# OSU-slatelab/ASR-CRaFT

Hardware: AMD Instinct MI355X
Metric: utterances/sec SCRF forward-backward (TIMIT-shape) (higher is better)
Workload: dtype f64; 1 GPU; BASELINE config 2: segmental CRF forward-backward, 48 labels, max-seg-len 25, 39-dim x 300-frame utterances, stdstate map (lambda_len 18528); global_minibatch=4096, precision=fastlin, parallelism=dp1, rccl_ranks=0

## Files before the change

### asr-craft_amd/csrc/scrf_engine.cpp

```cpp
#include <dlfcn.h>
#include <time.h>
#include <unistd.h>
#include <stdarg.h>
#include <stdio.h>
#include <stdlib.h>
#include <string.h>

#include <algorithm>
#include <cmath>
#include <string>
#include <unordered_map>
#include <vector>

#include "scrf_kernels.h"

typedef struct { char internal[128]; } scrf_nccl_uid;
typedef void* scrf_nccl_comm;
struct RcclApi {
  void* lib = nullptr;
  int (*GetUniqueId)(scrf_nccl_uid*) = nullptr;
  int (*CommInitRank)(scrf_nccl_comm*, int, scrf_nccl_uid, int) = nullptr;
  int (*AllReduce)(const void*, void*, size_t, int, int, scrf_nccl_comm, hipStream_t) = nullptr;
  int (*CommDestroy)(scrf_nccl_comm) = nullptr;
  int (*GroupStart)() = nullptr;
// ... 55 lines not shown
  bool m0_valid = false;
  double* d_sums = nullptr;
  double* d_stage = nullptr;
  double* d_lamT[2] = {nullptr, nullptr};
  double* d_sums_stage = nullptr;
  int* d_latch = nullptr;
  int* h_latch = nullptr;
  double* h_sums = nullptr;
  hipEvent_t ev_sums = nullptr;
  bool sums_queued = false;
  hipEvent_t ev_status = nullptr;
  uint64_t n_lin_fallback = 0;
  char* scratch = nullptr;
  size_t scratch_cap = 0;
  hipStream_t stream2 = nullptr;
  struct PoolBlock { void* p; size_t cap; uint64_t epoch; };
  std::vector<PoolBlock> pool_free;
  std::unordered_map<void*, size_t> pool_cap;
  hipStream_t up_stream = nullptr;
  hipEvent_t pool_ev[8] = {nullptr, nullptr, nullptr, nullptr, nullptr, nullptr, nullptr, nullptr};
  uint64_t pool_epoch = 0, pool_done = 0;
  size_t pool_bytes = 0;
  char* scratch2 = nullptr;
  size_t scratch2_cap = 0;
  double* d_grad2 = nullptr;
  double* d_sums2 = nullptr;
  hipEvent_t ev_fork = nullptr, ev_join = nullptr;
  bool overlap_comm = false;
  bool early_done = false;
  uint64_t n_collectives = 0, n_overlapped = 0;
  double* d_pack = nullptr;
  void* d_rtab = nullptr;
  size_t rtab_bytes = 0;
  double* d_dtab = nullptr;
  double* d_sl_tab = nullptr;
  bool frame_mass = false;
  uint64_t n_post_split = 0, n_post_whole = 0;
  bool force_fb = false;
  double* d_w1 = nullptr;
  uint64_t n_decode_fix = 0, n_decode_fallback = 0;
  uint32_t *dec_lab = nullptr, *dec_n = nullptr, *dec_hlab = nullptr, *dec_hn = nullptr;
  float *dec_cost = nullptr, *dec_hcost = nullptr;
  uint64_t dec_cap_f = 0, dec_cap_u = 0;
  char* post_buf = nullptr;
  size_t post_cap = 0;
  scrf_arc* lp_arcs = nullptr;
  uint64_t lp_cap = 0;
  char* lp_meta = nullptr;
  size_t lp_meta_cap = 0;
  scrf_batch lp_batch = nullptr;
  std::vector<uint64_t> lp_off;
  uint64_t n_lp_calls = 0, n_lp_chunks = 0;
  uint32_t* al_ph = nullptr;
  uint64_t* al_off = nullptr;
  uint64_t al_cap_ph = 0, al_cap_u = 0;
  std::vector<uint64_t> al_bp_off;
  uint64_t n_al_calls = 0, n_al_chunks = 0, n_al_wave = 0, n_al_group = 0;
  uint32_t* tr_inv = nullptr;
  uint64_t tr_cap_inv = 0;
  std::vector<uint64_t> tr_cell_off;
  std::vector<uint32_t> tr_inv_h;
  uint64_t n_tr_calls = 0, n_tr_chunks = 0, n_tr_redone = 0;
  std::string err;
  struct KTime { std::string name; double ms; uint32_t n; };
  std::vector<KTime> ktimes;
  hipEvent_t kev[2] = {nullptr, nullptr};
// ... 187 lines not shown
  size_t nb = sizeof(double) * lay.lambda_len;
  CRCHK(hipMalloc((void**)&h->d_lambda, nb));
  CRCHK(hipMalloc((void**)&h->d_lambda_acc, nb));
  CRCHK(hipMalloc((void**)&h->d_gsa, nb));
  CRCHK(hipMalloc((void**)&h->d_grad, nb));
  CRCHK(hipMalloc((void**)&h->d_m0, sizeof(double) * lay.L * lay.L));
  CRCHK(hipMalloc((void**)&h->d_w1, sizeof(double) * lay.L));
  if (lay.D <= 40) CRCHK(hipMalloc((void**)&h->d_dtab, sizeof(double) * fused_dur_table_doubles(lay)));
  if (cfg->map_type >= SCRF_STDSPARSE) {
    if (lay.nsfe + lay.use_sb) CRCHK(hipMalloc((void**)&h->d_lamT[0], sizeof(double) * ((size_t)lay.nsfe + lay.use_sb) * lay.L));
    if (lay.ntfe + lay.use_tb) CRCHK(hipMalloc((void**)&h->d_lamT[1], sizeof(double) * ((size_t)lay.ntfe + lay.use_tb) * lay.L * lay.L));
  }
  if (cfg->model_type == SCRF_STDSEG && !lay.use_tf) CRCHK(hipMalloc((void**)&h->d_sl_tab, sizeof(double) * (2 * (size_t)lay.L * lay.L + 8)));
  CRCHK(hipMalloc((void**)&h->d_e0, sizeof(double) * lay.L * lay.L));
  CRCHK(hipMalloc((void**)&h->d_et0, sizeof(double) * lay.L * lay.L));
  CRCHK(hipMalloc((void**)&h->d_msh0, sizeof(double)));
  CRCHK(hipMalloc((void**)&h->d_sums, sizeof(double) * 8));
  CRCHK(hipMalloc((void**)&h->d_stage, nb));
  CRCHK(hipMalloc((void**)&h->d_sums_stage, sizeof(double) * 4));
  CRCHK(hipMalloc((void**)&h->d_latch, sizeof(int) * 2));
  CRCHK(hipHostMalloc((void**)&h->h_latch, sizeof(int) * 2, hipHostMallocDefault));
  h->h_latch[0] = h->h_latch[1] = 0;
  CRCHK(hipHostMalloc((void**)&h->h_sums, sizeof(double) * 4, hipHostMallocDefault));
  CRCHK(hipEventCreateWithFlags(&h->ev_sums, hipEventDisableTiming));
  CRCHK(hipEventCreateWithFlags(&h->ev_status, hipEventDisableTiming));
  CRCHK(hipEventCreate(&h->kev[0]));
  CRCHK(hipEventCreate(&h->kev[1]));
  CRCHK(hipMalloc((void**)&h->d_grad2, nb));
  CRCHK(hipMalloc((void**)&h->d_sums2, sizeof(double) * 4));
  CRCHK(hipStreamCreateWithFlags(&h->stream2, hipStreamNonBlocking));
  CRCHK(hipStreamCreateWithFlags(&h->up_stream, hipStreamNonBlocking));
  CRCHK(hipEventCreateWithFlags(&h->ev_fork, hipEventDisableTiming));
  CRCHK(hipEventCreateWithFlags(&h->ev_join, hipEventDisableTiming));
  CRCHK(hipMemsetAsync(h->d_lambda, 0, nb, h->stream));
  CRCHK(hipMemsetAsync(h->d_lambda_acc, 0, nb, h->stream));
  CRCHK(hipMemsetAsync(h->d_gsa, 0, nb, h->stream));
  CRCHK(hipMemsetAsync(h->d_grad, 0, nb, h->stream));
  CRCHK(hipMemsetAsync(h->d_sums, 0, sizeof(double) * 8, h->stream));
  for (int i = 0; i <= SCRF_N_PHASES; i++) {
    CRCHK(hipEventCreate(&h->ev[i][0]));
    CRCHK(hipEventCreate(&h->ev[i][1]));
  }
  h->ev_ok = true;
  CRCHK(hipStreamSynchronize(h->stream));
  if (h->shadow) {
    std::vector<double> z(h->xlay.lambda_len, 0.0);
    if (scrf_set_lambda(h, z.data(), h->xlay.lambda_len) != SCRF_OK) { g_create_err = h->err; scrf_destroy(h); return SCRF_ERR_HIP; }
  }
#undef CRCHK
  *out = h;
  return SCRF_OK;
}

extern "C" int scrf_destroy(scrf_handle h) {
  if (!h) return SCRF_OK;
  hipSetDevice(h->device);
  if (h->stream) hipStreamSynchronize(h->stream);
  if (h->comm && g_rccl.CommDestroy) g_rccl.CommDestroy(h->comm);
  hipFree(h->d_lambda); hipFree(h->d_lambda_acc); hipFree(h->d_gsa);
  if (h->own_grad) hipFree(h->d_grad);
  hipFree(h->d_grad2); hipFree(h->d_sums2); hipFree(h->scratch2);
  hipFree(h->d_stage); hipFree(h->d_sums_stage); hipFree(h->d_latch);
  hipFree(h->d_lamT[0]); hipFree(h->d_lamT[1]);
  if (h->h_latch) hipHostFree(h->h_latch);
  if (h->h_sums) hipHostFree(h->h_sums);
  if (h->ev_sums) hipEventDestroy(h->ev_sums);
  if (h->ev_status) hipEventDestroy(h->ev_status);
  if (h->kev[0]) hipEventDestroy(h->kev[0]);
  if (h->kev[1]) hipEventDestroy(h->kev[1]);
  if (h->stream2) { hipStreamSynchronize(h->stream2); hipStreamDestroy(h->stream2); }
  if (h->up_stream) { hipStreamSynchronize(h->up_stream); hipStreamDestroy(h->up_stream); }
  for (auto& bl : h->pool_free) hipFree(bl.p);
  for (auto& kv : h->pool_cap) hipFree(kv.first);
  for (int i = 0; i < 8; i++) if (h->pool_ev[i]) hipEventDestroy(h->pool_ev[i]);
  if (h->ev_fork) hipEventDestroy(h->ev_fork);
  if (h->ev_join) hipEventDestroy(h->ev_join);
  hipFree(h->dec_lab); hipFree(h->dec_n); hipFree(h->dec_cost);
  hipFree(h->al_ph); hipFree(h->al_off);
  hipFree(h->tr_inv);
  hipFree(h->post_buf);
  hipFree(h->lp_arcs); hipFree(h->lp_meta);
  if (h->dec_hlab) hipHostFree(h->dec_hlab);
  if (h->dec_hn) hipHostFree(h->dec_hn);
  if (h->dec_hcost) hipHostFree(h->dec_hcost);
  hipFree(h->d_w1); hipFree(h->d_dtab); hipFree(h->d_rtab); hipFree(h->d_pack); hipFree(h->d_sl_tab); hipFree(h->d_m0); hipFree(h->d_e0); hipFree(h->d_et0); hipFree(h->d_msh0); hipFree(h->d_sums); hipFree(h->scratch);
  if (h->ev_ok)
    for (int i = 0; i <= SCRF_N_PHASES; i++) { hipEventDestroy(h->ev[i][0]); hipEventDestroy(h->ev[i][1]); }
  if (h->own_stream && h->stream) hipStreamDestroy(h->stream);
  delete h;
  return SCRF_OK;
}

extern "C" const char* scrf_last_error(scrf_handle h) { return h ? h->err.c_str() : g_create_err.c_str(); }

extern "C" int scrf_set_stream(scrf_handle h, void* s) {
  if (!h) return SCRF_ERR_INVALID;
  HIPCHK(h, hipSetDevice(h->device));
  HIPCHK(h, hipStreamSynchronize(h->stream));
  if (h->own_stream) { hipStreamDestroy(h->stream); h->own_stream = false; }
  if (s) {
    h->stream = (hipStream_t)s;
  } else {
    HIPCHK(h, hipStreamCreateWithFlags(&h->stream, hipStreamNonBlocking));
    h->own_stream = true;
  }
  return SCRF_OK;
}

extern "C" int scrf_synchronize(scrf_handle h) {
// ... 834 lines not shown
    KT_RUN("k_windows", st, launch_windows(st, b->d_frames[s], b->d_sframe_off[s], bv, u0, u1, nfr, r.in_width, l.D, r.left_ctx, r.right_ctx,
                                           r.extract_seg_ftr, X, hybrid ? hybrid_row_floats(l, r.in_width) : l.F, col,
                                           (first_only ? 1 : 0) | (hybrid ? 2 : 0)));
  }
}

static bool ensure_m0(scrf_handle h, hipStream_t st) {
  if (h->m0_valid) return false;
  const ScrfLayout& l = h->lay;
  launch_scores_exact(st, nullptr, l.F, nullptr, 1, h->d_lambda, l, 1, l.L * l.L, h->d_m0);
  launch_exp_m(st, h->kn, h->d_m0, l.L, 1, h->d_e0, h->d_et0, h->d_msh0);
  h->m0_valid = true;
  return true;
}

static void relay_sparse_lambda(scrf_handle h, hipStream_t st) {
  launch_sp_relay(st, h->d_lambda, h->lay, 0, h->d_lamT[0]);
  if (h->lay.use_tf) launch_sp_relay(st, h->d_lambda, h->lay, 1, h->d_lamT[1]);
}

static int run_scores(scrf_handle h, scrf_batch b, uint32_t u0, uint32_t u1, ChunkBufs& cb, bool fast = false, int f32 = 0) {
  const ScrfLayout& l = h->lay;
  const uint64_t nfr = b->frame_off[u1] - b->frame_off[u0], nseg = b->seg_off[u1] - b->seg_off[u0];
  ScrfBatchView bv = b->view();
  if (cb.fused) {
    PhaseTimer tm(h, PH_SCORE, cb.st);
    const uint32_t W0 = b->recipe[0].in_width;
    ScrfFusedArgs fa = fused_args(h, b, u0, 0);
    if (h->d_dtab && h->kn.dtab) {
      launch_dur_table(cb.st, l, W0, h->d_lambda, h->d_dtab);
      fa.dtab = h->d_dtab;
      const size_t nb = fused_tile_table_bytes(l.D, fa.TB);
      if (nb > h->rtab_bytes) {
        hipFree(h->d_rtab); h->d_rtab = nullptr; h->rtab_bytes = 0;
        HIPCHK(h, hipMalloc(&h->d_rtab, nb));
        h->rtab_bytes = nb;
      }
      launch_tile_tables(cb.st, l.D, fa.TB, (cb.la && !cb.Wn) ? 1 : 0, h->d_rtab);
      if (h->kn.rtab) fa.rtab = h->d_rtab;
      fa.dma = h->kn.scores_dma ? 1 : 0;
    }
    if (pframe_supported(W0)) {
      KT_RUN("k_pframe", cb.st, launch_pframe(cb.st, b->d_frames[0] + b->frame_off[u0] * W0, W0, nfr, h->d_lambda, l, (cb.la ? 6 : 5) * l.L, cb.P));
      if (cb.la) KT_RUN("k_avg_prefix", cb.st, launch_avg_prefix(cb.st, bv, u0, u1 - u0, l.L, cb.P));
    } else {
      KT_RUN("k_scores_mfma(samples)", cb.st, launch_scores_mfma(cb.st, h->kn, b->d_frames[0] + b->frame_off[u0] * W0, W0, nullptr, nfr, h->d_lambda, l,
                         spec_samples(W0), (cb.la ? 6 : 5) * l.L, cb.P));
      if (cb.la) KT_RUN("k_avg_prefix", cb.st, launch_avg_prefix(cb.st, bv, u0, u1 - u0, l.L, cb.P));
    }
    if (cb.Wn) {
      launch_state_l1(cb.st, h->d_lambda, l, h->d_w1);
      HIPCHK(h, hipMemsetAsync(cb.fix_cnt, 0, sizeof(uint32_t), cb.st));
      ScrfDecodeOut dz;
      dz.wneg = cb.Wn; dz.w1 = h->d_w1; dz.xm_f = b->d_xm_f + b->frame_off[u0];
      dz.cnt = cb.fix_cnt; dz.list = cb.fix_list; dz.cap = cb.fix_cap;
      dz.bound_scale = h->kn.decode_bound_scale * 1.01 * 0x1p-53 * (double)(l.nsfe + 1 + 3 * W0 + 8);
      PhaseTimer tk(h, PH_K_SCORE, cb.st);
      KT_RUN("k_scores_fused(decode)", cb.st, launch_scores_fused_decode(cb.st, fa, l, h->d_lambda, cb.P, b->tile_off[0][u1] - b->tile_off[0][u0], dz));
      tk.stop(1);
      tm.stop(3);
      HIPCHK(h, hipGetLastError());
      return SCRF_OK;
    }
    cb.es_ready = cb.lin && l.L <= 48;
    {
      PhaseTimer tk(h, PH_K_SCORE, cb.st);
      KT_RUN("k_scores_fused", cb.st, launch_scores_fused(cb.st, fa, l, h->d_lambda, cb.P, b->tile_off[0][u1] - b->tile_off[0][u0], cb.S, f32,
                          cb.es_ready ? cb.smax : nullptr, cb.s_true, b->d_labels, cb.la ? 1 : 0));
      tk.stop(1);
    }
    tm.stop(2);
// ... 24 lines not shown
    KT_RUN("k_sp_scores(state)", cb.st, launch_sp_scores(cb.st, cb.X, l.F, nullptr, nseg, h->d_lamT[0], l, 0, cb.S));
    tk.stop(2);
    nl += 1;
    if (l.use_tf) {
      if (!cb.lamT_ready) launch_sp_relay(cb.st, h->d_lambda, l, 1, h->d_lamT[1]);
      launch_frame_rows(cb.st, bv, u0, u1, l.D, nfr, cb.xrow_cur, 0);
      KT_RUN("k_sp_scores(trans)", cb.st, launch_sp_scores(cb.st, cb.X, l.F, cb.xrow_cur, nfr, h->d_lamT[1], l, 1, cb.M));
      nl += 3;
    }
  } else if (!cb.fused) {
    PhaseTimer tk(h, PH_K_SCORE, cb.st);
    if (fast) KT_RUN("k_scores_mfma(state)", cb.st, launch_scores_mfma(cb.st, h->kn, cb.X, l.F, nullptr, nseg, h->d_lambda, l, scrf_spec_state(l), l.L, cb.S, f32));
    else KT_RUN("k_scores_exact(state)", cb.st, launch_scores_exact(cb.st, cb.X, l.F, nullptr, nseg, h->d_lambda, l, 0, l.L, cb.S));
    tk.stop(1);
  }
  if (sparse(h)) {
    if (!l.use_tf && ensure_m0(h, cb.st)) nl += 2;
  } else if (segtrans(h)) {
    if (fast) KT_RUN("k_scores_mfma(trans)", cb.st, launch_scores_mfma(cb.st, h->kn, cb.X, l.F, nullptr, nseg, h->d_lambda, l, scrf_spec_trans(l), l.L * l.L, cb.M, f32));
    else KT_RUN("k_scores_exact(trans)", cb.st, launch_scores_exact(cb.st, cb.X, l.F, nullptr, nseg, h->d_lambda, l, 1, l.L * l.L, cb.M));
    launch_zero_initial_rows(cb.st, bv, b->d_frame_u, u0, nfr, l.D, l.L, cb.M);
    nl += 2;
  } else if (l.use_tf) {
    launch_frame_rows(cb.st, bv, u0, u1, l.D, nfr, cb.xrow_cur, 0);
    if (fast) KT_RUN("k_scores_mfma(trans)", cb.st, launch_scores_mfma(cb.st, h->kn, cb.X, l.F, cb.xrow_cur, nfr, h->d_lambda, l, scrf_spec_trans(l), l.L * l.L, cb.M, f32));
    else KT_RUN("k_scores_exact(trans)", cb.st, launch_scores_exact(cb.st, cb.X, l.F, cb.xrow_cur, nfr, h->d_lambda, l, 1, l.L * l.L, cb.M));
    nl += 2;
  } else if (ensure_m0(h, cb.st)) nl += 2;
  tm.stop(nl);
  HIPCHK(h, hipGetLastError());
  return SCRF_OK;
}

static int run_dp(scrf_handle h, scrf_batch b, uint32_t u0, uint32_t u1, ChunkBufs& cb, bool post, uint32_t* nl_out, bool ponly = false) {
  const ScrfLayout& l = h->lay;
  const uint64_t nutt = u1 - u0, nfr = b->frame_off[u1] - b->frame_off[u0];
  const int frame_model = h->cfg.model_type == SCRF_STDFRAME || h->frame_mass;
  ScrfBatchView bv = b->view();
  uint32_t nl = 0;
  if (segtrans(h)) {
    if (fb_segtrans_smem_bytes(l, fb_block_threads(l)) > 160 * 1024)
      return fail(h, SCRF_ERR_INVALID, "labels x maximum duration = %u x %u is too large for the stdseg_no_dur recursion "
                  "(its three [D][L] rings must fit 160 KB of LDS)", l.L, l.D);
    KT_RUN("k_fb_segtrans", cb.st, launch_fb_segtrans(cb.st, h->kn, l, bv, u0, (uint32_t)nutt, b->d_prev_lab, cb.S, cb.M, cb.AD, cb.alpha, cb.beta,
                       post ? cb.XI : nullptr, b->d_numer, b->d_zx, b->d_status, post ? 1 : 0));
    nl = 1;
  } else if (!cb.wave) {
    if (fb_smem_bytes(l, fb_block_threads(l)) > 160 * 1024)
      return fail(h, SCRF_ERR_INVALID, "labels x maximum duration = %u x %u is too large for the workgroup-per-utterance recursion "
                  "(its two [D][L] rings must fit 160 KB of LDS; the wavefront kernels cover L <= 256 with D <= 40)", l.L, l.D);
    if (post && cb.xi_acc) HIPCHK(h, hipMemsetAsync(cb.xi_acc, 0, sizeof(double) * nutt * l.L * l.L, cb.st));
    KT_RUN("k_fb", cb.st, launch_fb(cb.st, l, bv, u0, (uint32_t)nutt, cb.S, cb.M, cb.m_per_frame, cb.AD, cb.alpha, cb.beta, post ? cb.XI : nullptr,
              post ? cb.xi_acc : nullptr, b->d_numer, b->d_zx, b->d_status, post ? 1 : 0, frame_model));
    nl = 1;
  } else {
    if (cb.m_per_frame) { KT_RUN("k_exp_m", cb.st, launch_exp_m(cb.st, h->kn, cb.M, l.L, nfr, cb.E, cb.ET, cb.msh)); nl++; }
    if (cb.lin) {
      const uint64_t nseg = b->seg_off[u1] - b->seg_off[u0];
      if (!cb.es_ready) {
        if (!ponly) KT_RUN("k_true_scores", cb.st, launch_true_scores(cb.st, l, bv, b->d_frame_u, u0, nfr, cb.S, cb.s_true));
        KT_RUN("k_exp_rows", cb.st, launch_exp_rows(cb.st, cb.S, nseg, l.L, cb.smax));
        nl += ponly ? 1 : 2;
      }
      {
        PhaseTimer tk(h, PH_K_DP, cb.st);
        KT_RUN(l.L > 64 ? "k_dp_lin_mw" : "k_dp_lin", cb.st, launch_dp_lin(cb.st, h->kn, l, bv, u0, (uint32_t)nutt, cb.S, cb.smax, cb.E, cb.ET, cb.msh, cb.m_per_frame, cb.dl,
                      b->d_zx, b->d_status));
        tk.stop(1);
      }
      if (ponly) {
        if (nl_out) *nl_out = nl + 1;
        HIPCHK(h, hipGetLastError());
        return SCRF_OK;
      }
      if (cb.fused) {
        if (l.L > 64) HIPCHK(h, hipMemsetAsync(cb.mass_s, 0, sizeof(double) * nfr, cb.st));
        uint32_t t_max = 0;
        for (uint64_t u = u0; u < u1; u++) t_max = std::max(t_max, b->T[u]);
        KT_RUN("k_post_z", cb.st, launch_post_z(cb.st, h->kn, l, bv, u0, (uint32_t)nutt, b->d_next_lab, cb.s_true, cb.M, cb.m_per_frame, cb.S, cb.smax,
                      cb.dl, b->d_zx, cb.numer_f, b->d_status, cb.Z, cb.mass_s, cb.la ? 1 : 0, t_max, nfr));
        cb.z_ready = true;
      } else {
        KT_RUN("k_post_lin", cb.st, launch_post_lin(cb.st, l, bv, b->d_frame_u, u0, nfr, b->d_next_lab, cb.s_true, cb.M, cb.m_per_frame, cb.S,
                        cb.smax, cb.dl, b->d_zx, cb.numer_f, b->d_status, cb.mass_s));
      }
      KT_RUN("k_mass_check", cb.st, launch_mass_check(cb.st, bv, b->d_frame_u, u0, nfr, l.L, frame_model, 1, cb.dl.a, cb.dl.ga, cb.dl.b, cb.dl.gb,
                        b->d_zx, cb.mass_s, b->d_status));
      KT_RUN("k_numer_reduce", cb.st, launch_numer_reduce(cb.st, bv, u0, (uint32_t)nutt, cb.numer_f, b->d_numer));
      if (l.use_tf) KT_RUN("k_xi_lin", cb.st, launch_xi_lin(cb.st, l, bv, b->d_frame_u, u0, nfr, cb.dl, b->d_zx));
      else KT_RUN("k_xi_scale", cb.st, launch_xi_scale(cb.st, bv, b->d_frame_u, u0, nfr, cb.dl, b->d_zx));
      nl += 5;
      if (l.use_tf) {
        KT_RUN("k_xi_full", cb.st, launch_xi_full(cb.st, l, bv, u0, u1, nfr, b->d_next_lab, cb.fA, cb.fB, cb.E, cb.msh, cb.XI));
        nl++;
      }
      if (nl_out) *nl_out = nl;
      HIPCHK(h, hipGetLastError());
      return SCRF_OK;
    }
    {
      PhaseTimer tk(h, PH_K_DP, cb.st);
      KT_RUN("k_dp_wave", cb.st, launch_dp_wave(cb.st, l, bv, u0, (uint32_t)nutt, cb.S, cb.E, cb.ET, cb.msh, cb.m_per_frame, cb.AD, cb.alpha,
                     cb.beta, cb.sd, b->d_zx, b->d_status));
      tk.stop(1);
    }
    nl++;
    if (post) {
      KT_RUN("k_post_state", cb.st, launch_post_state(cb.st, l, bv, u0, u1, nfr, b->d_next_lab, cb.S, cb.M, cb.m_per_frame, cb.AD, cb.beta,
                        b->d_zx, cb.numer_f, b->d_status, cb.mass_s));
      KT_RUN("k_mass_check", cb.st, launch_mass_check(cb.st, bv, b->d_frame_u, u0, nfr, l.L, frame_model, 0, cb.alpha, nullptr, cb.beta, nullptr,
                        b->d_zx, cb.mass_s, b->d_status));
      KT_RUN("k_numer_reduce", cb.st, launch_numer_reduce(cb.st, bv, u0, (uint32_t)nutt, cb.numer_f, b->d_numer));
      KT_RUN("k_xi_factors", cb.st, launch_xi_factors(cb.st, l, bv, u0, u1, nfr, cb.alpha, cb.sd, b->d_zx, cb.fA, cb.fB));
      nl += 4;
      if (l.use_tf) {
        KT_RUN("k_xi_full", cb.st, launch_xi_full(cb.st, l, bv, u0, u1, nfr, b->d_next_lab, cb.fA, cb.fB, cb.E, cb.msh, cb.XI));
        nl++;
      }
    }
  }
  if (nl_out) *nl_out = nl;
  HIPCHK(h, hipGetLastError());
  return SCRF_OK;
// ... 14 lines not shown
  latch[1] = SCRF_LATCH_IDLE;
}
static void latch_decode(const int* h_latch, int out[2]) {
  out[0] = out[1] = 0;
  if (h_latch[0] != 0 && h_latch[1] != SCRF_LATCH_IDLE) {
    out[0] = h_latch[1] & 0xff;
    out[1] = (int)((uint32_t)h_latch[1] >> 8);
  }
}
__global__ void k_commit(double* __restrict__ grad, const double* __restrict__ stage, uint32_t n,
                         double* __restrict__ sums, const double* __restrict__ sums_stage,
                         const int* __restrict__ latch) {
  if (latch[0] != 0) return;
  const uint32_t i = blockIdx.x * blockDim.x + threadIdx.x;
  if (i < n) grad[i] += stage[i];
  if (i < 3) sums[i] += sums_stage[i];
}

__global__ void k_commit_part(double* __restrict__ grad, const double* __restrict__ stage, uint32_t n, uint32_t stride, uint32_t nsf,
                              int part, double* __restrict__ sums, const double* __restrict__ sums_stage,
                              const int* __restrict__ latch) {
  if (latch[0] != 0) return;
  const uint32_t i = blockIdx.x * blockDim.x + threadIdx.x;
  if (i < n && ((i % stride >= nsf) ? 1 : 0) == part) grad[i] += stage[i];
  if (part == 0 && i < 3) sums[i] += sums_stage[i];
}

static const char* status_text(int code) {
  return code == SCRF_ERR_BAD_LABEL ? "the label is larger than nActualLabs*labMaxDur"
         : code == SCRF_ERR_EMPTY   ? "No features read from this sentence."
                                    : "overflow / NaN / log of zero in the recursion, or posterior-mass check failed";
}

static int queue_status(scrf_handle h, scrf_batch b) {
  hipLaunchKernelGGL(k_latch_status, dim3((b->U + 255) / 256), dim3(256), 0, h->stream, b->d_status, b->U, h->d_latch);
  HIPCHK(h, hipMemcpyAsync(h->h_latch, h->d_latch, sizeof(int) * 2, hipMemcpyDeviceToHost, h->stream));
  HIPCHK(h, hipEventRecord(h->ev_status, h->stream));
  return SCRF_OK;
}

static bool stdseg(scrf_handle h) { return h->cfg.model_type == SCRF_STDSEG; }
static uint32_t stdseg_La(scrf_handle h) { return h->lay.L / h->lay.D; }

struct StdsegBufs {
  float* X; uint32_t *row_t, *row_d, *row_u;
  double *S, *MX, *alpha, *beta, *G, *XI, *mass_s, *mass_t;
};
static void stdseg_layout(scrf_handle h, scrf_batch b, uint32_t u0, uint32_t u1, bool post, Arena& a, StdsegBufs* sb) {
  const ScrfLayout& l = h->lay;
  const uint32_t La = stdseg_La(h);
  const uint64_t nfr = b->frame_off[u1] - b->frame_off[u0], nseg = b->seg_off[u1] - b->seg_off[u0];
  memset(sb, 0, sizeof(*sb));
  sb->X = b->mode == 1 ? a.take<float>(nseg * l.F) : b->d_windows + b->seg_off[u0] * l.F;
  sb->row_t = a.take<uint32_t>(nseg); sb->row_d = a.take<uint32_t>(nseg); sb->row_u = a.take<uint32_t>(nseg);
  sb->S = a.take<double>(nseg * La); sb->alpha = a.take<double>(nseg * La); sb->beta = a.take<double>(nseg * La);
  sb->MX = a.take<double>(nseg * (size_t)l.L * La);
  if (post) {
    sb->G = a.take<double>(nseg * La); sb->XI = a.take<double>(nseg * (size_t)l.L * La);
    sb->mass_s = a.take<double>(nfr); sb->mass_t = a.take<double>(nfr);
  }
}
static size_t stdseg_chunk_size(scrf_handle h, scrf_batch b, uint32_t u0, uint32_t u1, bool post) {
  Arena m{nullptr, 0, 0};
  StdsegBufs sb;
  stdseg_layout(h, b, u0, u1, post, m, &sb);
  return m.off;
}
static bool stdseg_lin(scrf_handle h) {
  return h->kn.stdseg_lin && !h->force_fb && h->cfg.train_precision != SCRF_PREC_EXACT && h->lay.use_sf && stdseg_lin_supported(h->lay, stdseg_La(h));
}
static uint64_t sl_rows_per_chunk(uint64_t nfr) {
  uint64_t rpc = ((nfr + 255) / 256 + 31) & ~31ull;
// ... 222 lines not shown
  std::vector<uint32_t> cuts(1, 0);
  const bool two_lanes = h->kn.lanes > 1 && !h->timing && b->U >= 64;
  {
    const uint32_t cap = two_lanes ? (b->U + 3) / 4 : b->U;
    for (uint32_t u0 = 0; u0 < b->U;) {
      uint32_t u1 = plan_chunk(h, b, u0, nd);
      if (u1 - u0 > cap) u1 = u0 + cap;
      cuts.push_back(u1);
      u0 = u1;
    }
  }
  const size_t n_chunks = cuts.size() - 1;
  const bool use2 = two_lanes && n_chunks >= 2;
  if (!l.use_tf && !segtrans(h)) ensure_m0(h, h->stream);
  if (sparse(h)) relay_sparse_lambda(h, h->stream);
  if (use2) {
    HIPCHK(h, hipMemsetAsync(h->d_grad2, 0, sizeof(double) * l.lambda_len, h->stream));
    HIPCHK(h, hipMemsetAsync(h->d_sums2, 0, sizeof(double) * 4, h->stream));
    HIPCHK(h, hipEventRecord(h->ev_fork, h->stream));
    HIPCHK(h, hipStreamWaitEvent(h->stream2, h->ev_fork, 0));
  }
  for (size_t ci = 0; ci < n_chunks; ci++) {
    const uint32_t u0 = cuts[ci], u1 = cuts[ci + 1];
    const int lane = use2 ? (int)(ci & 1) : 0;
    ChunkBufs cb;
    int rc = carve(h, b, u0, u1, nd, &cb, lane);
    if (rc != SCRF_OK) return rc;
    if (!lane) { cb.grad = h->d_stage; cb.sums = h->d_sums_stage; }
    cb.lamT_ready = sparse(h);
    if (cb.lin) *used_lin = true;
    const uint64_t nutt = u1 - u0, nfr = b->frame_off[u1] - b->frame_off[u0], nseg = b->seg_off[u1] - b->seg_off[u0];
    rc = run_scores(h, b, u0, u1, cb, fast, f32);
    if (rc != SCRF_OK) return rc;
    {
      PhaseTimer tm(h, PH_FB, cb.st);
      uint32_t nl = 0;
      rc = run_dp(h, b, u0, u1, cb, true, &nl);
      if (rc != SCRF_OK) return rc;
      tm.stop(nl);
    }
    if (!use2 && ci + 1 == n_chunks) {
      rc = queue_status(h, b);
      if (rc != SCRF_OK) return rc;
    }
    const bool ov = h->overlap_comm && h->kn.comm_overlap && two_block_reduce(h) && !use2 && !h->timing && !sparse(h);
    bool trans_done = false;
    if (ov) {
      if (ci + 1 == n_chunks) {
        HIPCHK(h, hipEventSynchronize(h->ev_status));
        latch_decode(h->h_latch, latch);
        if (latch[0] == SCRF_ERR_NUMERIC && wave_path(h, true)) return SCRF_OK;
      }
      launch_frame_rows(cb.st, bv, u0, u1, l.D, nfr, cb.xrow_next, 1);
      if (fast) launch_expf_mfma(cb.st, h->kn, cb.XI, l.L * l.L, cb.X, l.F, cb.xrow_next, nfr, l, scrf_spec_trans(l), cb.rpc_t, cb.nch_t, cb.slab_t, f32);
      else launch_expf_gemm(cb.st, cb.XI, l.L * l.L, cb.X, l.F, cb.xrow_next, nfr, l, 1, cb.rpc_t, cb.nch_t, cb.slab_t);
      launch_reduce_slabs(cb.st, cb.slab_t, cb.nch_t, l.L * l.L, l, scrf_spec_trans(l), cb.grad);
      if (ci + 1 == n_chunks) {
        hipLaunchKernelGGL(k_commit_part, dim3((l.lambda_len + 255) / 256), dim3(256), 0, h->stream, h->d_grad, h->d_stage, l.lambda_len,
                           l.stride, l.nsf, 1, h->d_sums, h->d_sums_stage, h->d_latch);
        HIPCHK(h, hipEventRecord(h->ev_fork, h->stream));
        HIPCHK(h, hipStreamWaitEvent(h->stream2, h->ev_fork, 0));
        rc = allreduce_block(h, h->stream2, 1);
        if (rc != SCRF_OK) return rc;
        HIPCHK(h, hipEventRecord(h->ev_join, h->stream2));
        h->early_done = true;
      }
      trans_done = true;
    }
    bool side = false;
    uint32_t t_max = 0;
    if (cb.hybrid) for (uint64_t u = u0; u < u1; u++) t_max = std::max(t_max, b->T[u]);
    {
      PhaseTimer tm(h, PH_EXPF, cb.st);
      uint32_t nl = 1;
      if (cb.fused) {
        const uint32_t W0 = b->recipe[0].in_width;
        ScrfFusedArgs fa = fused_args(h, b, u0, cb.expf_plan.tile_list);
        side = h->kn.side && !use2 && !h->timing && cb.z_ready && pframe_supported(W0) && !l.use_tf && !segtrans(h) && cb.wave &&
               cb.expf_plan.ws;
        if (side) {
          HIPCHK(h, hipEventRecord(h->ev_fork, cb.st));
          HIPCHK(h, hipStreamWaitEvent(h->stream2, h->ev_fork, 0));
          launch_ztf(h->stream2, cb.Z, (cb.la ? 6 : 5) * l.L, b->d_frames[0] + b->frame_off[u0] * W0, W0, nfr, cb.rpc_l, cb.nch_l, cb.slab_l, 1);
          launch_reduce_slabs(h->stream2, cb.slab_l, cb.nch_l, (cb.la ? 6 : 5) * l.L, l, spec_samples(W0), cb.grad);
          launch_atb(h->stream2, l, cb.fA, cb.fB, nfr, cb.rpc_atb, cb.nch_atb, cb.slab_atb, h->d_m0, cb.grad, cb.lin ? cb.dl.gsd : nullptr);
          HIPCHK(h, hipEventRecord(h->ev_join, h->stream2));
        }
        {
          PhaseTimer tk(h, PH_K_EXPF, cb.st);
          KT_RUN("k_expf_fused", cb.st, launch_expf_fused(cb.st, h->kn, fa, l, cb.R, b->tile_off[cb.expf_plan.tile_list][u1] - b->tile_off[cb.expf_plan.tile_list][u0], cb.slab_s, cb.slab_d, f32, cb.la ? 1 : 0));
          tk.stop(1);
        }
        if (!cb.z_ready) KT_RUN("k_lin_z", cb.st, launch_lin_z(cb.st, l, bv, u0, (uint32_t)nutt, cb.R, cb.Z));
        if (!side && pframe_supported(W0))
          KT_RUN("k_ztf", cb.st, launch_ztf(cb.st, cb.Z, (cb.la ? 6 : 5) * l.L, b->d_frames[0] + b->frame_off[u0] * W0, W0, nfr, cb.rpc_l, cb.nch_l, cb.slab_l));
        else if (!side)
          KT_RUN("k_expf_mfma(samples)", cb.st, launch_expf_mfma(cb.st, h->kn, cb.Z, (cb.la ? 6 : 5) * l.L, b->d_frames[0] + b->frame_off[u0] * W0, W0, nullptr, nfr, l,
                           spec_samples(W0), cb.rpc_l, cb.nch_l, cb.slab_l));
        nl += 2;
      } else if (cb.hybrid) {
        const uint32_t W0 = b->recipe[0].in_width;
        {
          PhaseTimer tk(h, PH_K_EXPF, cb.st);
          KT_RUN("k_expf_mfma(state)", cb.st, launch_expf_mfma(cb.st, h->kn, cb.R, l.L, cb.X, hybrid_row_floats(l, W0), nullptr, nseg, l, spec_stats_x(l, W0), cb.rpc_s, cb.nch_s, cb.slab_s, f32));
          tk.stop(1);
        }
        KT_RUN("k_lin_z5", cb.st, launch_lin_z5(cb.st, l, bv, u0, (uint32_t)nutt, t_max, nfr, cb.R, cb.Z, cb.slab_d));
        if (pframe_supported(W0))
          KT_RUN("k_ztf", cb.st, launch_ztf(cb.st, cb.Z, 5 * l.L, b->d_frames[0] + b->frame_off[u0] * W0, W0, nfr, cb.rpc_l, cb.nch_l, cb.slab_l));
        else
          KT_RUN("k_expf_mfma(samples)", cb.st, launch_expf_mfma(cb.st, h->kn, cb.Z, 5 * l.L, b->d_frames[0] + b->frame_off[u0] * W0, W0, nullptr, nfr, l,
                           spec_samples(W0), cb.rpc_l, cb.nch_l, cb.slab_l));
        nl += 2;
      } else if (sparse(h)) {
        PhaseTimer tk(h, PH_K_EXPF, cb.st);
// ... 1392 lines not shown
```

### asr-craft_amd/csrc/scrf_fused.hip

```cpp
#include "scrf_dp_common.h"

#include <math.h>
#include <string.h>
#include <utility>
#include <type_traits>
#include <stdio.h>
#include <stdlib.h>

typedef double v4f64 __attribute__((ext_vector_type(4)));
typedef float v4f32 __attribute__((ext_vector_type(4)));

#define FU_GC 40
#define FU_XS 42
#define FU_WS 49
#define FU_ROWS SCRF_FUSED_ROWS_SCORES
#define FE_ROWS SCRF_FUSED_ROWS_EXPF
#define FE_RSF 80
#define FE_RS 48

__host__ __device__ inline uint32_t fu_sample_step(uint32_t d, int k) {
  const float ot = (float)((double)d * 0.1);
  return (uint32_t)ceilf(ot * (float)(2 * k + 1)) - 1u;
}
__device__ __forceinline__ uint32_t fu_div(uint32_t i, uint32_t magic) { return magic ? __umulhi(i, magic) : i; }
// ... 1682 lines not shown
    }
    FU_SETPRIO(0);
    fe_mfma_tile<NT, F32, xs, NKS>(Rs, Xs, wave, lk, li, n_ot, acc, acc32);
    FU_SETPRIO(1);
    __syncthreads();
    FU_STAMP(10);
    tile = ntile;
    ft = nft;
  }
  double* out = slab + (uint64_t)blockIdx.x * n_out * ncol;
#pragma unroll
  for (int j = 0; j < NT; j++) {
    const uint32_t q = wave + 4 * j;
    if (q >= n_ot) continue;
    const uint32_t n = q % 3, ct = q / 3;
    const uint32_t f = ct * 16 + li;
    if (f >= ncol) continue;
    const double sc = (lay.use_sb && f == 3 * W + D) ? lay.sbv : 1.0;
#pragma unroll
    for (int r = 0; r < 4; r++) {
      const uint32_t o = o0 + n * 16 + (F32 ? 4 * lk + r : lk + 4 * r);
      if (o >= n_out) continue;
      const double v = F32 ? (double)acc32[F32 ? j : 0][r] : acc[F32 ? 0 : j][r];
      out[(uint64_t)o * ncol + f] = v * sc;
    }
  }
}

#define FW_NT 512
#define FW_DSL 5
#ifndef FW_DMA_NT
#define FW_DMA_NT 1
#endif
__device__ __forceinline__ void fw_dma16(uint32_t voff, const void* sbase, uint32_t lds) { fu_dma<16, FW_DMA_NT>(voff, sbase, lds); }
template <int NT, int DMAX, int NKS, int G0, int ROWS, int DMA>
__device__ __forceinline__ void expf_fused_ws_body(const ScrfFusedArgs& fa, const ScrfLayout& lay, const double* __restrict__ R,
                                                   uint32_t n_out, uint64_t n_tiles, uint32_t n_ct,
                                                   double* __restrict__ slab, double* __restrict__ dslab) {
  extern __shared__ __attribute__((aligned(16))) unsigned char fsm[];
  const uint32_t W = fa.W, D = lay.D;
  constexpr uint32_t xs = (NT == 4 ? 5 : NT <= 7 ? 9 : 13) * 16;
  constexpr uint32_t XB = (ROWS + 1) * xs;
  constexpr uint32_t RB = ROWS * FE_RS;
  constexpr int NRP = (ROWS * 48 + 255) / 256;
  constexpr int NDQ = (ROWS * 24 + 255) / 256;
  float* Xs0 = (float*)fsm;
  double* Rs0 = (double*)(Xs0 + 2 * XB);
  const uint32_t tid = threadIdx.x, lane = tid & 63;
  const uint32_t wave = __builtin_amdgcn_readfirstlane(tid >> 6);
  const bool producer = wave >= 4;
  const uint32_t li = lane & 15, lk = lane >> 4;
  const uint32_t o0 = blockIdx.y * 48;
  const uint32_t st0 = G0 + (gridDim.z > 1 ? blockIdx.z : 0u);
  const uint32_t ngrp = gridDim.z > 1 ? 1u : (uint32_t)(3 - G0);
  const uint32_t ncol = ngrp * W, ncol_all = (3 - G0) * W, zoff = gridDim.z > 1 ? blockIdx.z * W : 0u;
  const uint32_t n_ot = 3 * n_ct;
  for (uint32_t i = tid; i < 2 * XB; i += FW_NT) Xs0[i] = 0.0f;
  for (uint32_t i = tid; i < 2 * RB; i += FW_NT) Rs0[i] = 0.0;

  v4f64 acc[NT];
  v4f32 acc32_unused[1];
#pragma unroll
  for (int j = 0; j < NT; j++) acc[j] = (v4f64){0.0, 0.0, 0.0, 0.0};

  const uint64_t first = (gridDim.y == 1 && gridDim.z == 1) ? xcd_swizzle(blockIdx.x, gridDim.x) : blockIdx.x;
  const uint64_t G = gridDim.x;
// ... 53 lines not shown
      for (int q = 0; q < NDQ; q++) {
        const uint32_t c = ptid + 256 * q, row = c / 24, pr = c - row * 24;
        if (FU_ABL != 5 && row < ft.nrows && pr < npr) fw_dma16(row * rowb + pr * 16u, Rt, Rw + q * 4096u);
      }
      if (sum_buf < 2) dur_sums(sum_buf);
    } else {
#pragma unroll
    for (int q = 0; q < NRP; q++) {
      const uint32_t e = ptid + 256 * q, row = e / 48, ol = e % 48;
      const double* Rt = R + ft.row0 * n_out + o0;
      const uint32_t offb = (row * n_out + ol) * 8u;
      rp[q] = (FU_ABL != 5 && row < ft.nrows && o0 + ol < n_out) ? __builtin_nontemporal_load((const double*)((const char*)Rt + offb)) : 0.0;
    }
    if (sum_buf < 2) dur_sums(sum_buf);
    }
    {
      const float* gfr = fa.frames + (fa.frame_base + ft.fr0) * (uint64_t)W;
      const uint32_t nfW = ft.nfr * W, mfW = fu_magic(nfW);
      const bool full = FU_FULLSCAN && D == (uint32_t)DMAX && ft.t0 + 1 >= D;
      float* dump = Xs + ROWS * xs;
      auto decode = [&](uint32_t i, uint32_t& st, uint32_t& tl, uint32_t& c) {
        const uint32_t g = fu_div(i, mfW);
        st = g + st0;
        const uint32_t rem = i - g * nfW;
        tl = fu_div(rem, mW);
        c = rem - tl * W;
      };
      auto scan_full = [&](const float (&v)[DMAX], uint32_t st, float* o) {
        if (G0 == 0 && st == 0) fu_scan_avg_full<DMAX, xs>(v, o);
        else if (st == 1) fu_scan_ext_full<DMAX, 1, xs>(v, o);
        else fu_scan_ext_full<DMAX, 0, xs>(v, o);
      };
      if (FU_ABL == 6) {
      } else if (G0 == 1 && ngrp == 2 && full) {
        const uint32_t per = (nfW + 3) >> 2, pw = ptid >> 6, pl = ptid & 63;
        for (uint32_t j = pl; j < per; j += 64) {
          const uint32_t i = pw * per + j;
          if (i < nfW) {
            const uint32_t tl = fu_div(i, mW), c = i - tl * W;
            float v[DMAX];
            fu_load_vals_full<DMAX>(gfr, (ft.t0 + tl - ft.f0) * W + c, W, v);
            float* o = Xs + tl * (DMAX * xs) + c;
            float amx = v[0], amn = v[0];
#pragma unroll
            for (int jj = 0; jj < DMAX; jj++) {
              amx = fu_vmax(amx, v[jj]);
              amn = fu_vmin(amn, v[jj]);
              o[jj * xs] = amx;
              o[jj * xs + W] = amn;
            }
          }
        }
      } else
      for (uint32_t i0 = ptid; i0 < ngrp * nfW; i0 += 512) {
        const uint32_t i1 = i0 + 256;
        const bool two = i1 < ngrp * nfW;
        uint32_t st0_, tl0, c0, st1, tl1, c1;
        decode(i0, st0_, tl0, c0);
        decode(two ? i1 : i0, st1, tl1, c1);
        if (full) {
          float v0[DMAX], v1[DMAX];
          fu_load_vals_full<DMAX>(gfr, (ft.t0 + tl0 - ft.f0) * W + c0, W, v0);
          fu_load_vals_full<DMAX>(gfr, (ft.t0 + tl1 - ft.f0) * W + c1, W, v1);
          scan_full(v0, st0_, Xs + tl0 * (DMAX * xs) + (st0_ - st0) * W + c0);
          if (two) scan_full(v1, st1, Xs + tl1 * (DMAX * xs) + (st1 - st0) * W + c1);
        } else {
// ... 282 lines not shown
```

Measured before the change: 145,600 utterances/s.

## Cache tile tables, move post-DP checks to side stream, split producer scan

```diff
diff --git a/asr-craft_amd/csrc/scrf_engine.cpp b/asr-craft_amd/csrc/scrf_engine.cpp
--- a/asr-craft_amd/csrc/scrf_engine.cpp
+++ b/asr-craft_amd/csrc/scrf_engine.cpp
@@ -111,6 +111,10 @@
   double* d_pack = nullptr;
   void* d_rtab = nullptr;
   size_t rtab_bytes = 0;
+  uint32_t rtab_key[3] = {0, 0, 0};
+  bool rtab_valid = false;
+  hipStream_t rtab_stream = nullptr;
+  hipEvent_t ev_rtab = nullptr;
   double* d_dtab = nullptr;
   double* d_sl_tab = nullptr;
   bool frame_mass = false;
@@ -364,6 +368,7 @@
   CRCHK(hipStreamCreateWithFlags(&h->up_stream, hipStreamNonBlocking));
   CRCHK(hipEventCreateWithFlags(&h->ev_fork, hipEventDisableTiming));
   CRCHK(hipEventCreateWithFlags(&h->ev_join, hipEventDisableTiming));
+  CRCHK(hipEventCreateWithFlags(&h->ev_rtab, hipEventDisableTiming));
   CRCHK(hipMemsetAsync(h->d_lambda, 0, nb, h->stream));
   CRCHK(hipMemsetAsync(h->d_lambda_acc, 0, nb, h->stream));
   CRCHK(hipMemsetAsync(h->d_gsa, 0, nb, h->stream));
@@ -407,6 +412,7 @@
   for (int i = 0; i < 8; i++) if (h->pool_ev[i]) hipEventDestroy(h->pool_ev[i]);
   if (h->ev_fork) hipEventDestroy(h->ev_fork);
   if (h->ev_join) hipEventDestroy(h->ev_join);
+  if (h->ev_rtab) hipEventDestroy(h->ev_rtab);
   hipFree(h->dec_lab); hipFree(h->dec_n); hipFree(h->dec_cost);
   hipFree(h->al_ph); hipFree(h->al_off);
   hipFree(h->tr_inv);
@@ -1307,11 +1313,18 @@
       fa.dtab = h->d_dtab;
       const size_t nb = fused_tile_table_bytes(l.D, fa.TB);
       if (nb > h->rtab_bytes) {
-        hipFree(h->d_rtab); h->d_rtab = nullptr; h->rtab_bytes = 0;
+        hipFree(h->d_rtab); h->d_rtab = nullptr; h->rtab_bytes = 0; h->rtab_valid = false;
         HIPCHK(h, hipMalloc(&h->d_rtab, nb));
         h->rtab_bytes = nb;
       }
-      launch_tile_tables(cb.st, l.D, fa.TB, (cb.la && !cb.Wn) ? 1 : 0, h->d_rtab);
+      const uint32_t key[3] = {l.D, fa.TB, (cb.la && !cb.Wn) ? 1u : 0u};
+      if (!h->rtab_valid || memcmp(key, h->rtab_key, sizeof(key)) != 0) {
+        launch_tile_tables(cb.st, key[0], key[1], (int)key[2], h->d_rtab);
+        HIPCHK(h, hipEventRecord(h->ev_rtab, cb.st));
+        memcpy(h->rtab_key, key, sizeof(key));
+        h->rtab_valid = true;
+        h->rtab_stream = cb.st;
+      } else if (cb.st != h->rtab_stream) HIPCHK(h, hipStreamWaitEvent(cb.st, h->ev_rtab, 0));
       if (h->kn.rtab) fa.rtab = h->d_rtab;
       fa.dma = h->kn.scores_dma ? 1 : 0;
     }
@@ -1402,7 +1415,9 @@
   return SCRF_OK;
 }
 
-static int run_dp(scrf_handle h, scrf_batch b, uint32_t u0, uint32_t u1, ChunkBufs& cb, bool post, uint32_t* nl_out, bool ponly = false) {
+static int queue_status(scrf_handle h, scrf_batch b, hipStream_t st);
+static int run_dp(scrf_handle h, scrf_batch b, uint32_t u0, uint32_t u1, ChunkBufs& cb, bool post, uint32_t* nl_out, bool ponly = false,
+                  bool side_checks = false, bool status_too = false) {
   const ScrfLayout& l = h->lay;
   const uint64_t nutt = u1 - u0, nfr = b->frame_off[u1] - b->frame_off[u0];
   const int frame_model = h->cfg.model_type == SCRF_STDFRAME || h->frame_mass;
@@ -1454,11 +1469,21 @@
         KT_RUN("k_post_lin", cb.st, launch_post_lin(cb.st, l, bv, b->d_frame_u, u0, nfr, b->d_next_lab, cb.s_true, cb.M, cb.m_per_frame, cb.S,
                         cb.smax, cb.dl, b->d_zx, cb.numer_f, b->d_status, cb.mass_s));
       }
-      KT_RUN("k_mass_check", cb.st, launch_mass_check(cb.st, bv, b->d_frame_u, u0, nfr, l.L, frame_model, 1, cb.dl.a, cb.dl.ga, cb.dl.b, cb.dl.gb,
+      hipStream_t ck = cb.st;
+      if (side_checks) {
+        HIPCHK(h, hipEventRecord(h->ev_fork, cb.st));
+        HIPCHK(h, hipStreamWaitEvent(h->stream2, h->ev_fork, 0));
+        ck = h->stream2;
+      }
+      KT_RUN("k_mass_check", ck, launch_mass_check(ck, bv, b->d_frame_u, u0, nfr, l.L, frame_model, 1, cb.dl.a, cb.dl.ga, cb.dl.b, cb.dl.gb,
                         b->d_zx, cb.mass_s, b->d_status));
-      KT_RUN("k_numer_reduce", cb.st, launch_numer_reduce(cb.st, bv, u0, (uint32_t)nutt, cb.numer_f, b->d_numer));
-      if (l.use_tf) KT_RUN("k_xi_lin", cb.st, launch_xi_lin(cb.st, l, bv, b->d_frame_u, u0, nfr, cb.dl, b->d_zx));
-      else KT_RUN("k_xi_scale", cb.st, launch_xi_scale(cb.st, bv, b->d_frame_u, u0, nfr, cb.dl, b->d_zx));
+      KT_RUN("k_numer_reduce", ck, launch_numer_reduce(ck, bv, u0, (uint32_t)nutt, cb.numer_f, b->d_numer));
+      if (l.use_tf) KT_RUN("k_xi_lin", ck, launch_xi_lin(ck, l, bv, b->d_frame_u, u0, nfr, cb.dl, b->d_zx));
+      else KT_RUN("k_xi_scale", ck, launch_xi_scale(ck, bv, b->d_frame_u, u0, nfr, cb.dl, b->d_zx));
+      if (side_checks && status_too) {
+        int rc = queue_status(h, b, ck);
+        if (rc != SCRF_OK) return rc;
+      }
       nl += 5;
       if (l.use_tf) {
         KT_RUN("k_xi_full", cb.st, launch_xi_full(cb.st, l, bv, u0, u1, nfr, b->d_next_lab, cb.fA, cb.fB, cb.E, cb.msh, cb.XI));
@@ -1539,12 +1564,13 @@
                                     : "overflow / NaN / log of zero in the recursion, or posterior-mass check failed";
 }
 
-static int queue_status(scrf_handle h, scrf_batch b) {
-  hipLaunchKernelGGL(k_latch_status, dim3((b->U + 255) / 256), dim3(256), 0, h->stream, b->d_status, b->U, h->d_latch);
-  HIPCHK(h, hipMemcpyAsync(h->h_latch, h->d_latch, sizeof(int) * 2, hipMemcpyDeviceToHost, h->stream));
-  HIPCHK(h, hipEventRecord(h->ev_status, h->stream));
-  return SCRF_OK;
-}
+static int queue_status(scrf_handle h, scrf_batch b, hipStream_t st) {
+  hipLaunchKernelGGL(k_latch_status, dim3((b->U + 255) / 256), dim3(256), 0, st, b->d_status, b->U, h->d_latch);
+  HIPCHK(h, hipMemcpyAsync(h->h_latch, h->d_latch, sizeof(int) * 2, hipMemcpyDeviceToHost, st));
+  HIPCHK(h, hipEventRecord(h->ev_status, st));
+  return SCRF_OK;
+}
+static int queue_status(scrf_handle h, scrf_batch b) { return queue_status(h, b, h->stream); }
 
 static bool stdseg(scrf_handle h) { return h->cfg.model_type == SCRF_STDSEG; }
 static uint32_t stdseg_La(scrf_handle h) { return h->lay.L / h->lay.D; }
@@ -1833,18 +1859,20 @@
     const uint64_t nutt = u1 - u0, nfr = b->frame_off[u1] - b->frame_off[u0], nseg = b->seg_off[u1] - b->seg_off[u0];
     rc = run_scores(h, b, u0, u1, cb, fast, f32);
     if (rc != SCRF_OK) return rc;
+    const bool ov = h->overlap_comm && h->kn.comm_overlap && two_block_reduce(h) && !use2 && !h->timing && !sparse(h);
+    const bool side_pre = h->kn.side && !use2 && !h->timing && !ov && cb.fused && cb.lin && cb.wave && !l.use_tf && !segtrans(h) &&
+                          pframe_supported(b->recipe[0].in_width) && cb.expf_plan.ws;
     {
       PhaseTimer tm(h, PH_FB, cb.st);
       uint32_t nl = 0;
-      rc = run_dp(h, b, u0, u1, cb, true, &nl);
+      rc = run_dp(h, b, u0, u1, cb, true, &nl, false, side_pre, ci + 1 == n_chunks);
       if (rc != SCRF_OK) return rc;
       tm.stop(nl);
     }
-    if (!use2 && ci + 1 == n_chunks) {
+    if (!use2 && !side_pre && ci + 1 == n_chunks) {
       rc = queue_status(h, b);
       if (rc != SCRF_OK) return rc;
     }
-    const bool ov = h->overlap_comm && h->kn.comm_overlap && two_block_reduce(h) && !use2 && !h->timing && !sparse(h);
     bool trans_done = false;
     if (ov) {
       if (ci + 1 == n_chunks) {
@@ -1877,11 +1905,8 @@
       if (cb.fused) {
         const uint32_t W0 = b->recipe[0].in_width;
         ScrfFusedArgs fa = fused_args(h, b, u0, cb.expf_plan.tile_list);
-        side = h->kn.side && !use2 && !h->timing && cb.z_ready && pframe_supported(W0) && !l.use_tf && !segtrans(h) && cb.wave &&
-               cb.expf_plan.ws;
+        side = side_pre;
         if (side) {
-          HIPCHK(h, hipEventRecord(h->ev_fork, cb.st));
-          HIPCHK(h, hipStreamWaitEvent(h->stream2, h->ev_fork, 0));
           launch_ztf(h->stream2, cb.Z, (cb.la ? 6 : 5) * l.L, b->d_frames[0] + b->frame_off[u0] * W0, W0, nfr, cb.rpc_l, cb.nch_l, cb.slab_l, 1);
           launch_reduce_slabs(h->stream2, cb.slab_l, cb.nch_l, (cb.la ? 6 : 5) * l.L, l, spec_samples(W0), cb.grad);
           launch_atb(h->stream2, l, cb.fA, cb.fB, nfr, cb.rpc_atb, cb.nch_atb, cb.slab_atb, h->d_m0, cb.grad, cb.lin ? cb.dl.gsd : nullptr);
diff --git a/asr-craft_amd/csrc/scrf_fused.hip b/asr-craft_amd/csrc/scrf_fused.hip
--- a/asr-craft_amd/csrc/scrf_fused.hip
+++ b/asr-craft_amd/csrc/scrf_fused.hip
@@ -1738,6 +1738,10 @@
 #ifndef FW_DMA_NT
 #define FW_DMA_NT 1
 #endif
+#ifndef FW_SCAN
+#define FW_SCAN 1
+#endif
+constexpr bool fw_scan_split(int rows) { return FW_SCAN == 2 || (FW_SCAN == 1 && rows <= 76); }
 __device__ __forceinline__ void fw_dma16(uint32_t voff, const void* sbase, uint32_t lds) { fu_dma<16, FW_DMA_NT>(voff, sbase, lds); }
 template <int NT, int DMAX, int NKS, int G0, int ROWS, int DMA>
 __device__ __forceinline__ void expf_fused_ws_body(const ScrfFusedArgs& fa, const ScrfLayout& lay, const double* __restrict__ R,
@@ -1857,6 +1861,17 @@
         else fu_scan_ext_full<DMAX, 0, xs>(v, o);
       };
       if (FU_ABL == 6) {
+      } else if (fw_scan_split(ROWS) && G0 == 1 && ngrp == 2 && full) {
+        const uint32_t pw = wave - 4, half = (nfW + 1) >> 1, pl = ptid & 63;
+        const uint32_t lo = (pw & 1) ? half : 0u, hi = (pw & 1) ? nfW : half;
+        for (uint32_t i = lo + pl; i < hi; i += 64) {
+          const uint32_t tl = fu_div(i, mW), c = i - tl * W;
+          float v[DMAX];
+          fu_load_vals_full<DMAX>(gfr, (ft.t0 + tl - ft.f0) * W + c, W, v);
+          float* o = Xs + tl * (DMAX * xs) + c;
+          if (pw < 2) fu_scan_ext_full<DMAX, 1, xs>(v, o);
+          else fu_scan_ext_full<DMAX, 0, xs>(v, o + W);
+        }
       } else if (G0 == 1 && ngrp == 2 && full) {
         const uint32_t per = (nfW + 3) >> 2, pw = ptid >> 6, pl = ptid & 63;
         for (uint32_t j = pl; j < per; j += 64) {
```

Result: faster. 148,000 utterances/s, median of 6 (+1.6%).
